# Bluear7878/Remote-Sensing-Vision-Language-Diffusion-Model

Measured on AMD Instinct MI355X. Metric: 512px x8 SR images/sec @50 steps, higher is better.
Workload: dtype f16 / bf16 MFMA operands as hi + lo pairs and triples, f32 accumulation and f32 residual streams (Stage 1: f16 tensors x f16 weight pairs; Stage 2: rsvld_amd.ops.UNET_POLICY; config.precision) -- the composition inside 1e-3 of the reference's CPU path (config.tolerance)

## Files before the change

include/rsvld_hip.h:

```cpp
#ifndef RSVLD_HIP_H
#define RSVLD_HIP_H

#include <stdint.h>

#ifdef __cplusplus
extern "C" {
#endif

#define RSVLD_OK 0
#define RSVLD_EINVAL (-1)
#define RSVLD_EUNSUPPORTED (-2)
#define RSVLD_ELAUNCH (-3)

#define RSVLD_F16 0
#define RSVLD_BF16 1
#define RSVLD_F32 2
#define RSVLD_SPLIT 3
#define RSVLD_F16W2 4
#define RSVLD_F16Q8 6
#define RSVLD_F16W1 5

#define RSVLD_ACT_NONE 0
#define RSVLD_ACT_SILU 1
#define RSVLD_ACT_GEGLU 2
// ... 167 lines not shown
int rsvld_llama_decode_attention(const void* qkv, const void* cos, const void* sin, const int64_t* pos, void* kcache, void* vcache, void* out,
                                 float* ws, int n_q, int n_kv, int head_dim, int max_len, float scale, int dtype, void* stream);

int rsvld_split_planes(const float* x, void* planes, int64_t rows, int C, void* stream);
int rsvld_merge_planes(const void* planes, float* x, int64_t rows, int C, void* stream);
int rsvld_planes_to_f16(const void* planes, int64_t ld, int64_t plane_stride, void* out_f16, int64_t out_ld, int64_t rows, int C, void* stream);
int rsvld_f16_to_planes(const void* x_f16, int64_t ld, void* planes, int64_t rows, int C, void* stream);
int rsvld_split_pack_weights(const float* w, void* w3, int64_t Cout, int taps, int Ctot, void* stream);
int rsvld_pack_weight_pairs(const float* w, void* w2, int64_t Cout, int taps, int Ctot, void* stream);
int rsvld_pack_weight_hq8(const float* w, void* whq, int64_t Cout, int taps, int Ctot, void* stream);
int rsvld_split_hq8(const float* x, void* out, int64_t rows, int C, void* stream);
int rsvld_planes_transpose_triple(const void* planes, void* w3, int64_t rows, int64_t rows_p, int C, int64_t ld, void* stream);
int rsvld_planes_to_triple(const void* planes, void* w3, int64_t rows, int64_t rows_p, int C, int64_t ld, void* stream);
int rsvld_softmax_rows_split(const float* s, void* p_planes, int64_t rows, int cols, int cols_p, int64_t ld, float scale, void* stream);
int rsvld_groupnorm_scale_shift_f32(const float* x, const float* x2, const float* gamma, const float* beta, float* scale_shift,
                                    int B, int HW, int C1, int C2, int groups, float eps, void* ws, void* stream);
int rsvld_groupnorm_stats_f32_fast(const float* x, const float* x2, float* mean_var, int B, int HW, int C1, int C2, int groups,
                                   void* ws, void* stream);
int rsvld_groupnorm_scale_shift_from_stats(const float* mean_var, const float* gamma, const float* beta, float* scale_shift,
                                           int B, int C, int groups, float eps, void* stream);
int rsvld_groupnorm_apply_split(const float* x, const float* x2, void* out, const float* scale_shift,
                                const float* mod_scale1p, const float* mod_shift, int mod_stride,
                                int B, int HW, int C1, int C2, int silu, int out_f32, void* stream);
int rsvld_layernorm_split(const float* x, void* out, const float* gamma, const float* beta, int64_t rows, int C, float eps,
                          int out_f32, void* stream);
int rsvld_attention_split_d64(const void* q, const void* k, const void* v, void* out, int B, int heads, int Nq, int Nk,
                              int64_t q_batch_stride, int64_t q_tok_stride, int64_t q_plane,
                              int64_t k_batch_stride, int64_t k_tok_stride, int64_t k_plane,
                              int64_t v_batch_stride, int64_t v_tok_stride, int64_t v_plane,
                              int64_t o_batch_stride, int64_t o_tok_stride, int64_t o_plane,
                              float scale, int out_f32, void* stream);
int rsvld_attention_split_d512_shared(const void* q, const void* x, void* out, int B, int Nq, int Nk,
                                      int64_t q_batch_stride, int64_t q_tok_stride, int64_t q_plane,
                                      int64_t x_batch_stride, int64_t x_tok_stride, int64_t x_plane,
                                      int64_t o_batch_stride, int64_t o_tok_stride, int64_t o_plane,
                                      float scale, int out_f32, void* stream);

#ifdef __cplusplus
}
#endif
#endif
```

remote-sensing-vision-language-diffusion-model_amd/_lib.py:

```python
import ctypes as C
import os

_PKG_DIR = os.path.dirname(os.path.abspath(__file__))
LIB_PATH = os.environ.get("RSVLD_LIB") or os.path.join(_PKG_DIR, "librsvld_hip.so")

F16, BF16, F32 = 0, 1, 2
SPLIT = 3
F16W2 = 4
F16W1 = 5
F16Q8 = 6
ACT_NONE, ACT_SILU, ACT_GEGLU = 0, 1, 2
TUNE_TILE = {"256x64": 1, "128x64": 2, "128x128": 3, "64x128": 4}
TUNE_STAGES_SHIFT, TUNE_NO_KSPLIT, TUNE_REG_STAGING = 3, 1 << 6, 1 << 7
TUNE_HALO_NW4, TUNE_HALO_NW8, TUNE_NO_GEMM256 = 1 << 8, 1 << 9, 1 << 10
TUNE_GEMM_ONE_TILE = 1 << 12
TUNE_F32_SPLIT = 1 << 11

ERRORS = {-1: "RSVLD_EINVAL (bad shape / pointer / combination)",
          -2: "RSVLD_EUNSUPPORTED", -3: "RSVLD_ELAUNCH (HIP launch failed)"}


class RsvldError(RuntimeError):
    pass

# ... 68 lines not shown
    "rsvld_concat_c_f32": (_i, [_vp, _vp, _vp, _i64, _i, _i, _vp]),
    "rsvld_axpby_f32": (_i, [_vp, _vp, _vp, _i64, _f, _f, _vp]),
    "rsvld_absdiff_sums_f32": (_i, [_vp, _vp, _vp, _i, _i64, _vp]),
    "rsvld_attention_f32": (_i, [_vp, _vp, _vp, _vp, _i, _i, _i, _i, _i,
                                 _i64, _i64, _i64, _i64, _i64, _i64, _i64, _i64, _f, _vp]),
    "rsvld_attention_f32_split": (_i, [_vp, _vp, _vp, _vp, _i, _i, _i, _i, _i,
                                 _i64, _i64, _i64, _i64, _i64, _i64, _i64, _i64, _f, _vp]),
    "rsvld_nchw_f32_to_nhwc_f32": (_i, [_vp, _vp, _i, _i, _i, _i, _i, _i, _i, _f, _vp]),
    "rsvld_split_planes": (_i, [_vp, _vp, _i64, _i, _vp]),
    "rsvld_merge_planes": (_i, [_vp, _vp, _i64, _i, _vp]),
    "rsvld_planes_to_f16": (_i, [_vp, _i64, _i64, _vp, _i64, _i64, _i, _vp]),
    "rsvld_f16_to_planes": (_i, [_vp, _i64, _vp, _i64, _i, _vp]),
    "rsvld_split_pack_weights": (_i, [_vp, _vp, _i64, _i, _i, _vp]),
    "rsvld_pack_weight_pairs": (_i, [_vp, _vp, _i64, _i, _i, _vp]),
    "rsvld_pack_weight_hq8": (_i, [_vp, _vp, _i64, _i, _i, _vp]),
    "rsvld_split_hq8": (_i, [_vp, _vp, _i64, _i, _vp]),
    "rsvld_planes_transpose_triple": (_i, [_vp, _vp, _i64, _i64, _i, _i64, _vp]),
    "rsvld_planes_to_triple": (_i, [_vp, _vp, _i64, _i64, _i, _i64, _vp]),
    "rsvld_softmax_rows_split": (_i, [_vp, _vp, _i64, _i, _i, _i64, _f, _vp]),
    "rsvld_groupnorm_scale_shift_f32": (_i, [_vp, _vp, _vp, _vp, _vp, _i, _i, _i, _i, _i, _f, _vp, _vp]),
    "rsvld_groupnorm_stats_f32_fast": (_i, [_vp, _vp, _vp, _i, _i, _i, _i, _i, _vp, _vp]),
    "rsvld_groupnorm_scale_shift_from_stats": (_i, [_vp, _vp, _vp, _vp, _i, _i, _i, _f, _vp]),
    "rsvld_groupnorm_apply_split": (_i, [_vp, _vp, _vp, _vp, _vp, _vp, _i, _i, _i, _i, _i, _i, _i, _vp]),
    "rsvld_layernorm_split": (_i, [_vp, _vp, _vp, _vp, _i64, _i, _f, _i, _vp]),
    "rsvld_attention_split_d512_shared": (_i, [_vp, _vp, _vp, _i, _i, _i, _i64, _i64, _i64, _i64, _i64, _i64, _i64, _i64, _i64, _f, _i, _vp]),
    "rsvld_attention_split_d64": (_i, [_vp, _vp, _vp, _vp, _i, _i, _i, _i,
                                       _i64, _i64, _i64, _i64, _i64, _i64, _i64, _i64, _i64, _i64, _i64, _i64, _f, _i, _vp]),
}

_lib = None


def load():
    global _lib
    if _lib is not None:
        return _lib
    import torch
    if not os.path.exists(LIB_PATH):
        raise RsvldError(
            f"{LIB_PATH} not found: build it with `python -c 'import __graft_entry__ as g; g.build()'` "
            f"(or `make -C {os.path.join(_PKG_DIR, 'csrc')}`). There is no CPU fallback.")
    lib = C.CDLL(LIB_PATH)
    for name, (res, args) in SIGNATURES.items():
        fn = getattr(lib, name)
        fn.restype = res
        fn.argtypes = args
# ... 8 lines not shown
```

remote-sensing-vision-language-diffusion-model_amd/csrc/norm.hip:

```cpp
#include "rsvld_common.h"

namespace {

template <typename T>
__global__ __launch_bounds__(256) void gn_partial_kernel(const T* __restrict__ x1, const T* __restrict__ x2,
                                                         float* __restrict__ part, int HW, int C1, int C2,
                                                         int groups, int rows_per_chunk, int nchunks) {
    extern __shared__ __attribute__((aligned(16))) char smem_raw[];
    float* sm = (float*)smem_raw;
    const int C = C1 + C2, C8 = C >> 3, C1_8 = C1 >> 3;
    const int TPR = C8 < 256 ? C8 : 256;
    const int rif = 256 / TPR;
    const int tid = threadIdx.x;
    const int chunk = blockIdx.x, b = blockIdx.y;
    const int row_lo = chunk * rows_per_chunk;
    const int row_hi = min(HW, row_lo + rows_per_chunk);
    const int tc = tid % TPR, rsub = tid / TPR;
    if (rsub < rif) {
        for (int cc = tc; cc < C8; cc += TPR) {
            float s[8], ss[8];
#pragma unroll
            for (int e = 0; e < 8; ++e) { s[e] = 0.f; ss[e] = 0.f; }
            const T* src;
            int64_t cstride;
// ... 57 lines not shown
        ss += __shfl_xor(ss, o);
    }
    if (lane == 0) {
        const double mean = s * inv_count;
        double var = ss * inv_count - mean * mean;
        if (var < 0.0) var = 0.0;
        stats[2 * i] = (float)mean;
        stats[2 * i + 1] = (float)var;
    }
}

template <bool PER_CHANNEL>
__global__ __launch_bounds__(256) void gn_ab_kernel(const float* __restrict__ part1, int n1, int C1,
                                                    const float* __restrict__ part2, int n2, int C2,
                                                    const float* __restrict__ gamma, const float* __restrict__ beta,
                                                    float* __restrict__ ab, float* __restrict__ stats_out, int groups,
                                                    float eps, double inv_count) {
    __shared__ double red[2][4];
    __shared__ float mr[2];
    const int g = blockIdx.x, b = blockIdx.y, tid = threadIdx.x;
    const int C = C1 + C2, gs = C / groups;
    double s = 0.0, ss = 0.0;
    if (PER_CHANNEL) {
        for (int c = g * gs; c < (g + 1) * gs; ++c) {
            const float* base;
            int n, Cs, cc;
            if (c < C1) { base = part1 + (int64_t)b * n1 * C1 * 2; n = n1; Cs = C1; cc = c; }
            else { base = part2 + (int64_t)b * n2 * C2 * 2; n = n2; Cs = C2; cc = c - C1; }
            for (int t = tid; t < n; t += 256) {
                s += (double)base[((int64_t)t * Cs + cc) * 2];
                ss += (double)base[((int64_t)t * Cs + cc) * 2 + 1];
            }
        }
    } else {
        for (int t = tid; t < n1; t += 256) {
            const float* q = part1 + (((int64_t)b * n1 + t) * groups + g) * 2;
            s += (double)q[0];
            ss += (double)q[1];
        }
    }
#pragma unroll
    for (int o = 32; o > 0; o >>= 1) { s += __shfl_xor(s, o); ss += __shfl_xor(ss, o); }
    if ((tid & 63) == 0) { red[0][tid >> 6] = s; red[1][tid >> 6] = ss; }
    __syncthreads();
    if (tid == 0) {
        s = red[0][0] + red[0][1] + red[0][2] + red[0][3];
        ss = red[1][0] + red[1][1] + red[1][2] + red[1][3];
        const double mean = s * inv_count;
        double var = ss * inv_count - mean * mean;
        if (var < 0.0) var = 0.0;
        mr[0] = (float)mean;
        mr[1] = (float)var;
        if (stats_out != nullptr) {
            stats_out[((int64_t)b * groups + g) * 2] = (float)mean;
// ... 218 lines not shown
#pragma unroll
            for (int e = 0; e < 8; ++e) {
                const float t = f[e] * sa[e] + sb[e];
                f[e] = silu ? silu_f(t) : t;
            }
            *(u32x4*)(dst + (int64_t)(row0 + i * rstep) * C) = pack8<T>(f);
        }
}


__device__ __forceinline__ void ld8f(const float* p, float (&f)[8]) {
    const f32x4 a = *(const f32x4*)p, b = *(const f32x4*)(p + 4);
    f[0] = a[0]; f[1] = a[1]; f[2] = a[2]; f[3] = a[3]; f[4] = b[0]; f[5] = b[1]; f[6] = b[2]; f[7] = b[3];
}
__device__ __forceinline__ void st_planes8(bf16* row, int C, int c, const float (&f)[8]) {
    bf16x8 hv;
    float lo[8];
#pragma unroll
    for (int e = 0; e < 8; ++e) { hv[e] = (bf16)f[e]; lo[e] = f[e] - (float)hv[e]; }
    *(u32x4*)(row + c) = pack8<bf16>(lo);
    *(u32x4*)(row + C + c) = __builtin_bit_cast(u32x4, hv);
}

__global__ __launch_bounds__(256) void gn_partial_f32_kernel(const float* __restrict__ x1, const float* __restrict__ x2,
                                                             float* __restrict__ part, int HW, int C1, int C2, int groups,
                                                             int rows_per_chunk, int nchunks) {
    extern __shared__ __attribute__((aligned(16))) char smem_raw[];
    float* sm = (float*)smem_raw;
    const int C = C1 + C2, C8 = C >> 3, C1_8 = C1 >> 3;
    const int TPR = C8 < 256 ? C8 : 256, rif = 256 / TPR;
    const int tid = threadIdx.x, chunk = blockIdx.x, b = blockIdx.y;
    const int row_lo = chunk * rows_per_chunk, row_hi = min(HW, row_lo + rows_per_chunk);
    const int tc = tid % TPR, rsub = tid / TPR;
    if (rsub < rif) {
        for (int cc = tc; cc < C8; cc += TPR) {
            float s[8], ss[8];
#pragma unroll
            for (int e = 0; e < 8; ++e) { s[e] = 0.f; ss[e] = 0.f; }
            const float* src;
            int64_t cstride;
            int coff;
            if (cc < C1_8) { src = x1 + (int64_t)b * HW * C1; cstride = C1; coff = cc * 8; }
            else { src = x2 + (int64_t)b * HW * C2; cstride = C2; coff = (cc - C1_8) * 8; }
            int r = row_lo + rsub;
            for (; r + rif < row_hi; r += 2 * rif) {
                float f0[8], f1[8];
                ld8f(src + (int64_t)r * cstride + coff, f0);
                ld8f(src + (int64_t)(r + rif) * cstride + coff, f1);
#pragma unroll
                for (int e = 0; e < 8; ++e) { s[e] += f0[e]; ss[e] += f0[e] * f0[e]; }
#pragma unroll
                for (int e = 0; e < 8; ++e) { s[e] += f1[e]; ss[e] += f1[e] * f1[e]; }
            }
            for (; r < row_hi; r += rif) {
                float f[8];
                ld8f(src + (int64_t)r * cstride + coff, f);
#pragma unroll
                for (int e = 0; e < 8; ++e) { s[e] += f[e]; ss[e] += f[e] * f[e]; }
            }
            float* dst = sm + ((int64_t)rsub * C + cc * 8) * 2;
#pragma unroll
            for (int e = 0; e < 8; ++e) { dst[2 * e] = s[e]; dst[2 * e + 1] = ss[e]; }
        }
    }
    __syncthreads();
    const int gs = C / groups;
    for (int g = tid; g < groups; g += 256) {
        float s = 0.f, ss = 0.f;
        for (int r = 0; r < rif; ++r) {
            const float* src = sm + ((int64_t)r * C + g * gs) * 2;
            for (int e = 0; e < gs; ++e) { s += src[2 * e]; ss += src[2 * e + 1]; }
        }
        float* o = part + (((int64_t)b * nchunks + chunk) * groups + g) * 2;
        o[0] = s;
        o[1] = ss;
    }
}

template <int OUT>
__global__ __launch_bounds__(256) void gn_apply_split_kernel(const float* __restrict__ x1, const float* __restrict__ x2, void* __restrict__ y,
                                                             const float* __restrict__ ab, const float* __restrict__ mod_scale,
                                                             const float* __restrict__ mod_shift, int HW, int C1, int C2, int silu,
                                                             int rows_per_block, int mod_stride) {
    const int C = C1 + C2, C8 = C >> 3, C1_8 = C1 >> 3;
    const int TPR = C8 < 256 ? C8 : 256, rif = 256 / TPR;
    const int tid = threadIdx.x, tc = tid % TPR, rsub = tid / TPR;
    if (rsub >= rif) return;
    const int b = blockIdx.y;
    const int row_lo = blockIdx.x * rows_per_block, row_hi = min(HW, row_lo + rows_per_block);
    for (int cc = tc; cc < C8; cc += TPR) {
        float sa[8], sb[8];
        {
            const float* a = ab + ((int64_t)b * C + cc * 8) * 2;
#pragma unroll
            for (int e = 0; e < 8; ++e) { sa[e] = a[2 * e]; sb[e] = a[2 * e + 1]; }
        }
        const float* src;
        int64_t cstride;
        int coff;
        if (cc < C1_8) { src = x1 + (int64_t)b * HW * C1; cstride = C1; coff = cc * 8; }
        else { src = x2 + (int64_t)b * HW * C2; cstride = C2; coff = (cc - C1_8) * 8; }
        auto emit = [&](int r, float (&f)[8]) {
#pragma unroll
            for (int e = 0; e < 8; ++e) {
                const float t = f[e] * sa[e] + sb[e];
                f[e] = silu ? silu_f(t) : t;
            }
            if (mod_scale != nullptr) {
                const int64_t mo = ((int64_t)b * HW + r) * mod_stride + cc * 8;
                float ms[8], mh[8];
                ld8f(mod_scale + mo, ms);
                ld8f(mod_shift + mo, mh);
#pragma unroll
                for (int e = 0; e < 8; ++e) f[e] = f[e] * (1.f + ms[e]) + mh[e];
            }
            const int64_t pix = (int64_t)b * HW + r;
            if (OUT == 1) {
                float* o = (float*)y + pix * C + cc * 8;
                *(f32x4*)o = (f32x4){f[0], f[1], f[2], f[3]};
                *(f32x4*)(o + 4) = (f32x4){f[4], f[5], f[6], f[7]};
            } else if (OUT == 2) {
                *(u32x4*)((f16*)y + pix * C + cc * 8) = pack8<f16>(f);
            } else if (OUT == 3) {
                st_hq8<true, RSVLD_HQ8_SX_LO, RSVLD_HQ8_SX_HI>((f16*)y + pix * (2 * (int64_t)C), C, cc * 8, f);
            } else {
                st_planes8((bf16*)y + pix * (2 * C), C, cc * 8, f);
            }
        };
        int r = row_lo + rsub;
        for (; r + rif < row_hi; r += 2 * rif) {
            float f0[8], f1[8];
            ld8f(src + (int64_t)r * cstride + coff, f0);
            ld8f(src + (int64_t)(r + rif) * cstride + coff, f1);
            emit(r, f0);
            emit(r + rif, f1);
        }
        for (; r < row_hi; r += rif) {
            float f[8];
            ld8f(src + (int64_t)r * cstride + coff, f);
            emit(r, f);
        }
    }
}

template <int MAXC, int ROWS, int OUT>
__global__ __launch_bounds__(256) void layernorm_split_kernel(const float* __restrict__ x, void* __restrict__ y,
                                                              const float* __restrict__ gamma, const float* __restrict__ beta,
                                                              int64_t rows, int C, float eps) {
    const int lane = threadIdx.x & 63;
    const int C8 = C >> 3;
    float ga[MAXC][8], be[MAXC][8];
#pragma unroll
    for (int j = 0; j < MAXC; ++j) {
        const int cc = lane + 64 * j;
#pragma unroll
        for (int e = 0; e < 8; ++e) {
            ga[j][e] = (gamma != nullptr && cc < C8) ? gamma[cc * 8 + e] : 1.f;
            be[j][e] = (beta != nullptr && cc < C8) ? beta[cc * 8 + e] : 0.f;
        }
    }
    const int64_t wave_id = (int64_t)blockIdx.x * 4 + (threadIdx.x >> 6);
    const int64_t nwaves = (int64_t)gridDim.x * 4;
    for (int64_t row0 = wave_id * ROWS; row0 < rows; row0 += nwaves * ROWS) {
        float f[ROWS][MAXC][8];
// ... 58 lines not shown
    const float a = (gamma ? gamma[c] : 1.f) * (1.0f / sqrtf(var + eps));
    ab[2 * (int64_t)i] = a;
    ab[2 * (int64_t)i + 1] = (beta ? beta[c] : 0.f) - mean * a;
}

bool gn_small_ok(int B, int HW, int C1, int C2, int groups) {
    const int C = C1 + C2, gs = C / groups;
    if (gs % 8) return false;
    const int gs8 = gs / 8;
    if (gs8 > 256 || (gs8 & (gs8 - 1))) return false;
    if (C2 > 0 && C1 % gs) return false;
    if ((int64_t)HW * gs8 > (int64_t)256 * GN_SMALL_MAXV) return false;
    (void)B;
    return groups >= 32;
}

struct GnPlan {
    int nchunks, rows_per_chunk;
};
GnPlan gn_plan(int B, int HW) {
    (void)B;
    const int max_chunks = 512;
    int rpc = (HW + max_chunks - 1) / max_chunks;
    if (rpc < 64) rpc = 64;
    GnPlan p;
    p.rows_per_chunk = rpc;
    p.nchunks = (HW + rpc - 1) / rpc;
    return p;
}

bool gn_shape_ok(int B, int HW, int C1, int C2, int groups) {
    if (B <= 0 || HW <= 0 || C1 <= 0 || C1 % 8 || C2 < 0 || C2 % 8 || groups <= 0) return false;
    const int C = C1 + C2;
    if (C % groups) return false;
    if (C > 8192 || groups > 256) return false;
    return true;
}

template <typename T>
int gn_stats_impl(const void* x, const void* x2, float* stats, int B, int HW, int C1, int C2, int groups, void* ws,
                  hipStream_t s) {
    const GnPlan pl = gn_plan(B, HW);
    const int C = C1 + C2, C8 = C / 8;
    const int TPR = C8 < 256 ? C8 : 256, rif = 256 / TPR;
    const size_t smem = (size_t)rif * C * 2 * sizeof(float);
    float* part = (float*)ws;
// ... 140 lines not shown
    }
}

extern "C" int rsvld_layernorm(const void* x, void* y, const float* gamma, const float* beta, int64_t rows, int C,
                               float eps, int dtype, void* stream) {
    if (!x || !y || rows <= 0 || C <= 0 || C % 8 || C > 4096) return RSVLD_EINVAL;
    hipStream_t s = (hipStream_t)stream;
    if (dtype == RSVLD_F16) launch_layernorm<f16>(x, y, gamma, beta, rows, C, eps, s);
    else if (dtype == RSVLD_BF16) launch_layernorm<bf16>(x, y, gamma, beta, rows, C, eps, s);
    else return RSVLD_EINVAL;
    return rsvld_check_launch();
}

extern "C" int rsvld_groupnorm_scale_shift_f32(const float* x, const float* x2, const float* gamma, const float* beta,
                                               float* scale_shift, int B, int HW, int C1, int C2, int groups, float eps, void* ws,
                                               void* stream) {
    if (!x || !ws || !scale_shift || !gn_shape_ok(B, HW, C1, C2, groups) || ((C2 > 0) != (x2 != nullptr)) || B > 65535) return RSVLD_EINVAL;
    hipStream_t s = (hipStream_t)stream;
    const GnPlan pl = gn_plan(B, HW);
    const int C = C1 + C2, C8 = C / 8;
    const int TPR = C8 < 256 ? C8 : 256, rif = 256 / TPR;
    const size_t smem = (size_t)rif * C * 2 * sizeof(float);
    float* part = (float*)ws;
    hipLaunchKernelGGL(gn_partial_f32_kernel, dim3(pl.nchunks, B), dim3(256), smem, s, x, x2, part, HW, C1, C2, groups,
                       pl.rows_per_chunk, pl.nchunks);
    const double inv_count = 1.0 / ((double)HW * (double)(C / groups));
    hipLaunchKernelGGL(gn_ab_kernel<false>, dim3(groups, B), dim3(256), 0, s, part, pl.nchunks, C, nullptr, 0, 0, gamma, beta,
                       scale_shift, nullptr, groups, eps, inv_count);
    return rsvld_check_launch();
}

extern "C" int rsvld_groupnorm_apply_split(const float* x, const float* x2, void* out, const float* scale_shift,
                                           const float* mod_scale1p, const float* mod_shift, int mod_stride, int B, int HW, int C1,
                                           int C2, int silu, int out_f32, void* stream) {
    if (!x || !out || !scale_shift || B <= 0 || B > 65535 || HW <= 0 || C1 <= 0 || C1 % 8 || C2 < 0 || C2 % 8 || ((C2 > 0) != (x2 != nullptr)))
        return RSVLD_EINVAL;
    if ((mod_scale1p != nullptr) != (mod_shift != nullptr) || mod_stride < 0 || (mod_stride & 3)) return RSVLD_EINVAL;
    const int C = C1 + C2, C8 = C / 8;
    const int TPR = C8 < 256 ? C8 : 256, rif = 256 / TPR;
    int max_blocks = 2048 / B;
    if (max_blocks < 1) max_blocks = 1;
    int rpb = (HW + max_blocks - 1) / max_blocks;
    if (rpb < 2 * rif) rpb = 2 * rif;
    const int nblk = (HW + rpb - 1) / rpb;
    hipStream_t s = (hipStream_t)stream;
    if (out_f32 < 0 || out_f32 > 3 || (out_f32 == 3 && (C1 + C2) % 32)) return RSVLD_EINVAL;
    if (out_f32 == 3)
        hipLaunchKernelGGL(gn_apply_split_kernel<3>, dim3((unsigned)nblk, B), dim3(256), 0, s, x, x2, out, scale_shift, mod_scale1p,
                           mod_shift, HW, C1, C2, silu, rpb, mod_stride > 0 ? mod_stride : C);
    else if (out_f32 == 1)
        hipLaunchKernelGGL(gn_apply_split_kernel<1>, dim3((unsigned)nblk, B), dim3(256), 0, s, x, x2, out, scale_shift, mod_scale1p,
                           mod_shift, HW, C1, C2, silu, rpb, mod_stride > 0 ? mod_stride : C);
    else if (out_f32 == 2)
        hipLaunchKernelGGL(gn_apply_split_kernel<2>, dim3((unsigned)nblk, B), dim3(256), 0, s, x, x2, out, scale_shift, mod_scale1p,
                           mod_shift, HW, C1, C2, silu, rpb, mod_stride > 0 ? mod_stride : C);
    else
        hipLaunchKernelGGL(gn_apply_split_kernel<0>, dim3((unsigned)nblk, B), dim3(256), 0, s, x, x2, out, scale_shift, mod_scale1p,
                           mod_shift, HW, C1, C2, silu, rpb, mod_stride > 0 ? mod_stride : C);
    return rsvld_check_launch();
}

template <int OUT_F32>
static void launch_layernorm_split(const float* x, void* y, const float* gamma, const float* beta, int64_t rows, int C, float eps,
                                   hipStream_t s) {
    const int chunks_per_lane = (C / 8 + 63) / 64;
    auto blocks = [&](int rows_per_block) {
        const int64_t n = cdiv64(rows, rows_per_block);
        return (unsigned)(n < 768 ? n : 768);
    };
    if (chunks_per_lane <= 2) hipLaunchKernelGGL((layernorm_split_kernel<2, 2, OUT_F32>), dim3(blocks(8)), dim3(256), 0, s, x, y, gamma, beta, rows, C, eps);
    else if (chunks_per_lane == 3) hipLaunchKernelGGL((layernorm_split_kernel<3, 2, OUT_F32>), dim3(blocks(8)), dim3(256), 0, s, x, y, gamma, beta, rows, C, eps);
    else if (chunks_per_lane <= 4) hipLaunchKernelGGL((layernorm_split_kernel<4, 1, OUT_F32>), dim3(blocks(4)), dim3(256), 0, s, x, y, gamma, beta, rows, C, eps);
    else hipLaunchKernelGGL((layernorm_split_kernel<8, 1, OUT_F32>), dim3(blocks(4)), dim3(256), 0, s, x, y, gamma, beta, rows, C, eps);
}

extern "C" int rsvld_layernorm_split(const float* x, void* out, const float* gamma, const float* beta, int64_t rows, int C, float eps,
                                     int out_f32, void* stream) {
    if (!x || !out || rows <= 0 || C <= 0 || C % 8 || C > 4096) return RSVLD_EINVAL;
    hipStream_t s = (hipStream_t)stream;
    if (out_f32 < 0 || out_f32 > 2) return RSVLD_EINVAL;
    if (out_f32 == 1) launch_layernorm_split<1>(x, out, gamma, beta, rows, C, eps, s);
    else if (out_f32 == 2) launch_layernorm_split<2>(x, out, gamma, beta, rows, C, eps, s);
    else launch_layernorm_split<0>(x, out, gamma, beta, rows, C, eps, s);
    return rsvld_check_launch();
}

extern "C" int rsvld_groupnorm_stats_f32_fast(const float* x, const float* x2, float* mean_var, int B, int HW, int C1, int C2, int groups,
                                              void* ws, void* stream) {
    if (!x || !mean_var || !ws || !gn_shape_ok(B, HW, C1, C2, groups) || ((C2 > 0) != (x2 != nullptr)) || B > 65535) return RSVLD_EINVAL;
    hipStream_t s = (hipStream_t)stream;
    const GnPlan pl = gn_plan(B, HW);
    const int C = C1 + C2, C8 = C / 8;
    const int TPR = C8 < 256 ? C8 : 256, rif = 256 / TPR;
    const size_t smem = (size_t)rif * C * 2 * sizeof(float);
    float* part = (float*)ws;
    hipLaunchKernelGGL(gn_partial_f32_kernel, dim3(pl.nchunks, B), dim3(256), smem, s, x, x2, part, HW, C1, C2, groups,
                       pl.rows_per_chunk, pl.nchunks);
    const int total = B * groups;
    const double inv_count = 1.0 / ((double)HW * (double)(C / groups));
    hipLaunchKernelGGL(gn_finalize_kernel, dim3((total + 3) / 4), dim3(256), 0, s, part, mean_var, groups, pl.nchunks, inv_count, total);
    return rsvld_check_launch();
}

extern "C" int rsvld_groupnorm_scale_shift_from_stats(const float* mean_var, const float* gamma, const float* beta, float* scale_shift,
                                                      int B, int C, int groups, float eps, void* stream) {
    if (!mean_var || !scale_shift || B <= 0 || C <= 0 || groups <= 0 || C % groups) return RSVLD_EINVAL;
    const int total = B * C;
    hipLaunchKernelGGL(gn_ab_from_stats_kernel, dim3((total + 255) / 256), dim3(256), 0, (hipStream_t)stream, mean_var, gamma, beta,
                       scale_shift, C, groups, eps, total);
    return rsvld_check_launch();
}
```

remote-sensing-vision-language-diffusion-model_amd/ops.py:

```python
import contextlib
import ctypes as C
import contextvars
import math

import torch

from . import _lib as L

_DT = {torch.float16: L.F16, torch.bfloat16: L.BF16}


def _stream():
    return C.c_void_p(torch.cuda.current_stream().cuda_stream)


def _ptr(t):
    return None if t is None else C.c_void_p(t.data_ptr())


def _need_gpu(*ts):
    for t in ts:
        if t is not None and not t.is_cuda:
            raise L.RsvldError("rsvld_amd ops run on the GPU only (got a CPU tensor); there is no CPU fallback")

# ... 685 lines not shown
    lib = L.load()
    if not lib.rsvld_conv3x3_halo_supported(C.byref(d)):
        raise L.RsvldError("conv2d (q8): shape not supported by the halo kernel (checked by _q8_conv_eligible)")
    part_out, ntiles = None, ((H + 7) // 8) * ((W + 31) // 32)
    if stats:
        part_out = torch.empty((B, ntiles, pc.cout_p, 2), device=out.device, dtype=torch.float32)
    flops = 2.0 * B * H * W * pc.cout * pc.cin * 9
    nbytes = 4.0 * (B * H * W * Cc + out.numel() + (0 if residual is None else residual.numel())) + 4.0 * pc.w.numel()
    _launch("conv_halo_128_q8" + _detail(B, H, W, Cc, 0, pc, 1, False), flops, nbytes, lambda: L.check(
        lib.rsvld_conv3x3_halo_nhwc(C.byref(d), None, 0, _ptr(part_out), _stream()), "rsvld_conv3x3_halo_nhwc"))
    if part_out is not None:
        out._gn_part = (part_out, ntiles)
    out._nhwc = True
    return out


def _gn_scale_shift_f32(x, x2, gamma, nbeta, groups, eps):
    B, H, W, C1 = x.shape
    C2 = 0 if x2 is None else x2.shape[-1]
    lib = L.load()
    ab = torch.empty((B, C1 + C2, 2), device=x.device, dtype=torch.float32)
    part1 = getattr(x, "_gn_part", None)
    part2 = None if x2 is None else getattr(x2, "_gn_part", None)
    if part1 is not None and (x2 is None or part2 is not None):
        _launch("groupnorm_ab_from_partials", 0.0, 0.0, lambda: L.check(lib.rsvld_groupnorm_scale_shift_from_partials(
            _ptr(part1[0]), part1[1], C1, None if part2 is None else _ptr(part2[0]), 0 if part2 is None else part2[1],
            C2, _ptr(gamma), _ptr(nbeta), _ptr(ab), B, H * W, groups, eps, _stream()), "rsvld_groupnorm_scale_shift_from_partials"))
        return ab
    if not x.is_contiguous() or (x2 is not None and not x2.is_contiguous()):
        raise L.RsvldError("group_norm (split): contiguous fp32 NHWC inputs expected")
    ws = torch.empty(lib.rsvld_groupnorm_ws_bytes(B, H * W, C1 + C2, groups), device=x.device, dtype=torch.uint8)
    _launch("groupnorm_stats_split", 0.0, 4.0 * (x.numel() + (0 if x2 is None else x2.numel())), lambda: L.check(
        lib.rsvld_groupnorm_scale_shift_f32(_ptr(x), _ptr(x2), _ptr(gamma), _ptr(nbeta), _ptr(ab), B, H * W, C1, C2, groups, eps,
                                            _ptr(ws), _stream()), "rsvld_groupnorm_scale_shift_f32"))
    return ab


def _gn_apply_split(x, x2, ab, silu, planes, mod_scale1p=None, mod_shift=None, f16=False, q8=False):
    B, H, W, C1 = x.shape
    C2 = 0 if x2 is None else x2.shape[-1]
    Cc = C1 + C2
    mod_stride = 0
    if mod_scale1p is not None:
        mod_stride = mod_scale1p.stride(-2)
        if (mod_shift.stride(-2) != mod_stride or mod_scale1p.stride(-1) != 1 or mod_shift.stride(-1) != 1
                or mod_scale1p.dtype != torch.float32 or mod_shift.dtype != torch.float32):
            raise L.RsvldError("group_norm: modulation tensors must be fp32, share a row stride and be channel-contiguous")
    f16 = f16 and planes
    if q8:
        out = torch.empty((B, H, W, 2, Cc), device=x.device, dtype=torch.float16)
        _launch("groupnorm_apply_q8", 0.0, 8.0 * B * H * W * Cc, lambda: L.check(L.load().rsvld_groupnorm_apply_split(
            _ptr(x), _ptr(x2), _ptr(out), _ptr(ab), _ptr(mod_scale1p), _ptr(mod_shift), mod_stride, B, H * W, C1, C2, int(silu), 3, _stream()),
            "rsvld_groupnorm_apply_split"))
        return Q8Rows(out)
    if f16:
        out = torch.empty((B, H, W, Cc), device=x.device, dtype=torch.float16)
    elif planes:
        out = torch.empty((B, H, W, 2, Cc), device=x.device, dtype=torch.bfloat16)
    else:
        out = torch.empty((B, H, W, Cc), device=x.device, dtype=torch.float32)
    _launch("groupnorm_apply_split", 0.0, (6.0 if f16 else 8.0) * B * H * W * Cc, lambda: L.check(L.load().rsvld_groupnorm_apply_split(
        _ptr(x), _ptr(x2), _ptr(out), _ptr(ab), _ptr(mod_scale1p), _ptr(mod_shift), mod_stride, B, H * W, C1, C2, int(silu),
        2 if f16 else int(not planes), _stream()), "rsvld_groupnorm_apply_split"))
    if f16:
        return out
    if planes:
        return Planes(out)
    out._nhwc = True
    return out


def _detail(B, Ho, Wo, Cin, Cin2, pc, stride, upsample):
    if not _CTX.get().profile_detail:
        return ""
    return f" [{B}x{Ho}x{Wo} {Cin}+{Cin2}->{pc.cout_p} k{pc.kh} s{stride}{' up' if upsample else ''}]"


def _conv2d_split(x, pc, *, x2, stride, pad, upsample, rowvec, residual, act, alpha, beta, norm, stats, out_planes, out_group=None,
                  norm_group=None, group=None):

    if norm is not None:
        gamma, nbeta, groups, eps, silu = norm
        if isinstance(x, Planes) or isinstance(x2, Planes):
            raise L.RsvldError("conv2d (split): norm= needs the fp32 tensors")
        ab = _gn_scale_shift_f32(x, x2, gamma, nbeta, groups, eps)
        if f16_group(norm_group):
            x16 = _gn_apply_split(x, x2, ab, silu, planes=True, f16=True)
            return conv2d(x16, pc, stride=stride, pad=pad, upsample=upsample, rowvec=rowvec, residual=residual, act=act, alpha=alpha,
                          beta=beta, stats=stats, out_planes=out_planes, out_group=out_group, group=group)
        if q8_group(norm_group) and _q8_conv_eligible(x.shape[0], x.shape[1], x.shape[2], x.shape[3] + (0 if x2 is None else x2.shape[3]), pc,
                                                      stride, pad, upsample, act, out_planes):
            return _conv2d_q8(_gn_apply_split(x, x2, ab, silu, planes=True, q8=True), pc, rowvec=rowvec, residual=residual, alpha=alpha,
# ... 722 lines not shown
```

remote-sensing-vision-language-diffusion-model_amd/sgm/modules/diffusionmodules/openaimodel.py:

```python
import torch
from torch import nn

from .... import ops
from ....hipnn import HipNet
from ...util import default, exists
from ..attention import SpatialTransformer
from .util import conv_nd, linear, normalization, timestep_embedding, zero_module


class TimestepBlock(nn.Module):
    """Marker: ``run(rt, x, emb_rows)`` takes the timestep embedding."""


class TimestepEmbedSequential(nn.Sequential, TimestepBlock):
    def run(self, rt, x, emb_rows, context=None):
        for layer in self:
            if isinstance(layer, TimestepBlock):
                x = layer.run(rt, x, emb_rows)
            elif isinstance(layer, SpatialTransformer):
                x = layer.run(rt, x, context)
            elif isinstance(layer, nn.Conv2d):
                x = ops.conv2d(x, rt.pk(layer), pad=layer.padding[0])
            else:
                x = layer.run(rt, x)
# ... 39 lines not shown
        self.out_layers = nn.Sequential(normalization(self.out_channels), nn.SiLU(), nn.Dropout(p=dropout),
                                        zero_module(conv_nd(dims, self.out_channels, self.out_channels, kernel_size,
                                                            padding=pad)))
        if self.out_channels == channels:
            self.skip_connection = nn.Identity()
        elif use_conv:
            self.skip_connection = conv_nd(dims, channels, self.out_channels, kernel_size, padding=pad)
        else:
            self.skip_connection = conv_nd(dims, channels, self.out_channels, 1)

    @property
    def _emb_linear(self):
        return self.emb_layers[1]

    def run(self, rt, x, emb_rows):
        gn1, conv1 = self.in_layers[0], self.in_layers[2]
        gn2, conv2 = self.out_layers[0], self.out_layers[3]
        h = ops.conv2d(x, rt.pk(conv1), pad=conv1.padding[0], rowvec=emb_rows[id(self)], stats=True,
                       norm=(gn1.weight, gn1.bias, gn1.num_groups, gn1.eps, True), norm_group="conv1")
        if isinstance(self.skip_connection, nn.Conv2d):
            skip = ops.conv2d(x, rt.pk(self.skip_connection), pad=self.skip_connection.padding[0])
        else:
            skip = x
        return ops.conv2d(h, rt.pk(conv2), pad=conv2.padding[0], residual=skip,
                          norm=(gn2.weight, gn2.bias, gn2.num_groups, gn2.eps, True), norm_group="conv2")


class UNetModel(HipNet):

    def __init__(self, in_channels, model_channels, out_channels, num_res_blocks, attention_resolutions, dropout=0,
                 channel_mult=(1, 2, 4, 8), conv_resample=True, dims=2, num_classes=None, use_checkpoint=False,
                 use_fp16=False, num_heads=-1, num_head_channels=-1, num_heads_upsample=-1,
                 use_scale_shift_norm=False, resblock_updown=False, use_new_attention_order=False,
                 use_spatial_transformer=False, transformer_depth=1, context_dim=None, n_embed=None, legacy=True,
                 disable_self_attentions=None, num_attention_blocks=None, disable_middle_self_attn=False,
                 use_linear_in_transformer=False, spatial_transformer_attn_type="softmax", adm_in_channels=None,
                 use_fairscale_checkpoint=False, offload_to_cpu=False, transformer_depth_middle=None, **ignored):
        super().__init__()
        if not use_spatial_transformer or context_dim is None:
            raise NotImplementedError("the SR networks are SDXL UNets with spatial transformers")
        if resblock_updown or use_scale_shift_norm or n_embed is not None or dims != 2:
            raise NotImplementedError("option not used by juggernautXL.yaml")
        if num_heads == -1 and num_head_channels == -1:
            raise ValueError("Either num_heads or num_head_channels has to be set")
        channel_mult = list(channel_mult)
        if isinstance(context_dim, (list, tuple)):
            context_dim = list(context_dim)
# ... 100 lines not shown
```

Before: 0.01361.

## Fuse per-channel GroupNorm statistics into apply and conv epilogues, retune LayerNorm

The fp32 GroupNorm apply kernel now writes per-block per-channel sum and sum-of-squares partials, and the second ResBlock conv also requests stats. A following GroupNorm can then build scale and shift from these partials and skip a full re-read of the activation. When only one of two concatenated sources carries partials, the other source gets a partials-only pass. The partials reducer is vectorised and unrolled, and small-C LayerNorm gets a new wave-per-row-group kernel. The cost is extra partial-buffer writes and shared-memory reductions in the apply kernel, plus several interacting code paths to keep correct.

```diff
diff --git a/include/rsvld_hip.h b/include/rsvld_hip.h
--- a/include/rsvld_hip.h
+++ b/include/rsvld_hip.h
@@ -213,6 +213,11 @@
 int rsvld_groupnorm_apply_split(const float* x, const float* x2, void* out, const float* scale_shift,
                                 const float* mod_scale1p, const float* mod_shift, int mod_stride,
                                 int B, int HW, int C1, int C2, int silu, int out_f32, void* stream);
+int rsvld_groupnorm_row_blocks(int HW);
+int rsvld_groupnorm_apply_split_stats(const float* x, const float* x2, float* out, const float* scale_shift,
+                                      const float* mod_scale1p, const float* mod_shift, int mod_stride,
+                                      int B, int HW, int C1, int C2, int silu, float* part_out, void* stream);
+int rsvld_groupnorm_partials_f32(const float* x, float* part, int B, int HW, int C, void* stream);
 int rsvld_layernorm_split(const float* x, void* out, const float* gamma, const float* beta, int64_t rows, int C, float eps,
                           int out_f32, void* stream);
 int rsvld_attention_split_d64(const void* q, const void* k, const void* v, void* out, int B, int heads, int Nq, int Nk,
diff --git a/remote-sensing-vision-language-diffusion-model_amd/_lib.py b/remote-sensing-vision-language-diffusion-model_amd/_lib.py
--- a/remote-sensing-vision-language-diffusion-model_amd/_lib.py
+++ b/remote-sensing-vision-language-diffusion-model_amd/_lib.py
@@ -114,6 +114,9 @@
     "rsvld_groupnorm_stats_f32_fast": (_i, [_vp, _vp, _vp, _i, _i, _i, _i, _i, _vp, _vp]),
     "rsvld_groupnorm_scale_shift_from_stats": (_i, [_vp, _vp, _vp, _vp, _i, _i, _i, _f, _vp]),
     "rsvld_groupnorm_apply_split": (_i, [_vp, _vp, _vp, _vp, _vp, _vp, _i, _i, _i, _i, _i, _i, _i, _vp]),
+    "rsvld_groupnorm_row_blocks": (_i, [_i]),
+    "rsvld_groupnorm_apply_split_stats": (_i, [_vp, _vp, _vp, _vp, _vp, _vp, _i, _i, _i, _i, _i, _i, _vp, _vp]),
+    "rsvld_groupnorm_partials_f32": (_i, [_vp, _vp, _i, _i, _i, _vp]),
     "rsvld_layernorm_split": (_i, [_vp, _vp, _vp, _vp, _i64, _i, _f, _i, _vp]),
     "rsvld_attention_split_d512_shared": (_i, [_vp, _vp, _vp, _i, _i, _i, _i64, _i64, _i64, _i64, _i64, _i64, _i64, _i64, _i64, _f, _i, _vp]),
     "rsvld_attention_split_d64": (_i, [_vp, _vp, _vp, _vp, _i, _i, _i, _i,
diff --git a/remote-sensing-vision-language-diffusion-model_amd/csrc/norm.hip b/remote-sensing-vision-language-diffusion-model_amd/csrc/norm.hip
--- a/remote-sensing-vision-language-diffusion-model_amd/csrc/norm.hip
+++ b/remote-sensing-vision-language-diffusion-model_amd/csrc/norm.hip
@@ -103,14 +103,28 @@
     const int C = C1 + C2, gs = C / groups;
     double s = 0.0, ss = 0.0;
     if (PER_CHANNEL) {
-        for (int c = g * gs; c < (g + 1) * gs; ++c) {
-            const float* base;
-            int n, Cs, cc;
-            if (c < C1) { base = part1 + (int64_t)b * n1 * C1 * 2; n = n1; Cs = C1; cc = c; }
-            else { base = part2 + (int64_t)b * n2 * C2 * 2; n = n2; Cs = C2; cc = c - C1; }
-            for (int t = tid; t < n; t += 256) {
-                s += (double)base[((int64_t)t * Cs + cc) * 2];
-                ss += (double)base[((int64_t)t * Cs + cc) * 2 + 1];
+        const int W = gs < 256 ? gs : 256, nsub = 256 / W;
+        const int cl = tid % W, rsub = tid / W;
+        if (rsub < nsub) {
+            for (int c = g * gs + cl; c < (g + 1) * gs; c += W) {
+                const f32x2_t* p;
+                int n;
+                int64_t Cs;
+                if (c < C1) { p = (const f32x2_t*)part1 + (int64_t)b * n1 * C1 + c; n = n1; Cs = C1; }
+                else { p = (const f32x2_t*)part2 + (int64_t)b * n2 * C2 + (c - C1); n = n2; Cs = C2; }
+                int t = rsub;
+                for (; t + 3 * nsub < n; t += 4 * nsub) {
+                    f32x2_t v[4];
+#pragma unroll
+                    for (int u = 0; u < 4; ++u) v[u] = p[(int64_t)(t + u * nsub) * Cs];
+#pragma unroll
+                    for (int u = 0; u < 4; ++u) { s += (double)v[u][0]; ss += (double)v[u][1]; }
+                }
+                for (; t < n; t += nsub) {
+                    const f32x2_t v = p[(int64_t)t * Cs];
+                    s += (double)v[0];
+                    ss += (double)v[1];
+                }
             }
         }
     } else {
@@ -375,6 +389,7 @@
     *(u32x4*)(row + C + c) = __builtin_bit_cast(u32x4, hv);
 }
 
+template <bool PER_CHANNEL>
 __global__ __launch_bounds__(256) void gn_partial_f32_kernel(const float* __restrict__ x1, const float* __restrict__ x2,
                                                              float* __restrict__ part, int HW, int C1, int C2, int groups,
                                                              int rows_per_chunk, int nchunks) {
@@ -417,6 +432,15 @@
         }
     }
     __syncthreads();
+    if (PER_CHANNEL) {
+        float* o = part + ((int64_t)b * nchunks + chunk) * C * 2;
+        for (int i = tid; i < 2 * C; i += 256) {
+            float a = 0.f;
+            for (int r = 0; r < rif; ++r) a += sm[(int64_t)r * C * 2 + i];
+            o[i] = a;
+        }
+        return;
+    }
     const int gs = C / groups;
     for (int g = tid; g < groups; g += 256) {
         float s = 0.f, ss = 0.f;
@@ -430,18 +454,23 @@
     }
 }
 
-template <int OUT>
+template <int OUT, bool STATS>
 __global__ __launch_bounds__(256) void gn_apply_split_kernel(const float* __restrict__ x1, const float* __restrict__ x2, void* __restrict__ y,
                                                              const float* __restrict__ ab, const float* __restrict__ mod_scale,
-                                                             const float* __restrict__ mod_shift, int HW, int C1, int C2, int silu,
-                                                             int rows_per_block, int mod_stride) {
+                                                             const float* __restrict__ mod_shift, float* __restrict__ part_out, int HW,
+                                                             int C1, int C2, int silu, int rows_per_block, int mod_stride) {
+    static_assert(!STATS || OUT == 1, "statistics are those of the fp32 output");
+    __shared__ __attribute__((aligned(16))) float sm_part[STATS ? 256 * 16 : 1];
     const int C = C1 + C2, C8 = C >> 3, C1_8 = C1 >> 3;
     const int TPR = C8 < 256 ? C8 : 256, rif = 256 / TPR;
     const int tid = threadIdx.x, tc = tid % TPR, rsub = tid / TPR;
-    if (rsub >= rif) return;
+    if (!STATS && rsub >= rif) return;
     const int b = blockIdx.y;
     const int row_lo = blockIdx.x * rows_per_block, row_hi = min(HW, row_lo + rows_per_block);
-    for (int cc = tc; cc < C8; cc += TPR) {
+    for (int cc = tc; rsub < rif && cc < C8; cc += TPR) {
+        float ps[8], pss[8];
+#pragma unroll
+        for (int e = 0; e < 8; ++e) { ps[e] = 0.f; pss[e] = 0.f; }
         float sa[8], sb[8];
         {
             const float* a = ab + ((int64_t)b * C + cc * 8) * 2;
@@ -466,6 +495,10 @@
                 ld8f(mod_shift + mo, mh);
 #pragma unroll
                 for (int e = 0; e < 8; ++e) f[e] = f[e] * (1.f + ms[e]) + mh[e];
+            }
+            if (STATS) {
+#pragma unroll
+                for (int e = 0; e < 8; ++e) { ps[e] += f[e]; pss[e] += f[e] * f[e]; }
             }
             const int64_t pix = (int64_t)b * HW + r;
             if (OUT == 1) {
@@ -493,6 +526,26 @@
             ld8f(src + (int64_t)r * cstride + coff, f);
             emit(r, f);
         }
+        if (STATS) {
+            if (rif == 1) {
+                float* o = part_out + (((int64_t)b * gridDim.x + blockIdx.x) * C + cc * 8) * 2;
+#pragma unroll
+                for (int e = 0; e < 8; e += 2) *(f32x4*)(o + 2 * e) = (f32x4){ps[e], pss[e], ps[e + 1], pss[e + 1]};
+            } else {
+                float* o = sm_part + (rsub * C + cc * 8) * 2;
+#pragma unroll
+                for (int e = 0; e < 8; e += 2) *(f32x4*)(o + 2 * e) = (f32x4){ps[e], pss[e], ps[e + 1], pss[e + 1]};
+            }
+        }
+    }
+    if (STATS && rif > 1) {
+        __syncthreads();
+        float* o = part_out + ((int64_t)b * gridDim.x + blockIdx.x) * C * 2;
+        for (int i = tid; i < 2 * C; i += 256) {
+            float a = 0.f;
+            for (int r = 0; r < rif; ++r) a += sm_part[r * C * 2 + i];
+            o[i] = a;
+        }
     }
 }
 
@@ -597,6 +650,15 @@
     (void)B;
     const int max_chunks = 512;
     int rpc = (HW + max_chunks - 1) / max_chunks;
+    if (rpc < 64) rpc = 64;
+    GnPlan p;
+    p.rows_per_chunk = rpc;
+    p.nchunks = (HW + rpc - 1) / rpc;
+    return p;
+}
+
+GnPlan gn_pc_plan(int HW) {
+    int rpc = (HW + 2047) / 2048;
     if (rpc < 64) rpc = 64;
     GnPlan p;
     p.rows_per_chunk = rpc;
@@ -783,7 +845,7 @@
     const int TPR = C8 < 256 ? C8 : 256, rif = 256 / TPR;
     const size_t smem = (size_t)rif * C * 2 * sizeof(float);
     float* part = (float*)ws;
-    hipLaunchKernelGGL(gn_partial_f32_kernel, dim3(pl.nchunks, B), dim3(256), smem, s, x, x2, part, HW, C1, C2, groups,
+    hipLaunchKernelGGL(gn_partial_f32_kernel<false>, dim3(pl.nchunks, B), dim3(256), smem, s, x, x2, part, HW, C1, C2, groups,
                        pl.rows_per_chunk, pl.nchunks);
     const double inv_count = 1.0 / ((double)HW * (double)(C / groups));
     hipLaunchKernelGGL(gn_ab_kernel<false>, dim3(groups, B), dim3(256), 0, s, part, pl.nchunks, C, nullptr, 0, 0, gamma, beta,
@@ -807,18 +869,123 @@
     hipStream_t s = (hipStream_t)stream;
     if (out_f32 < 0 || out_f32 > 3 || (out_f32 == 3 && (C1 + C2) % 32)) return RSVLD_EINVAL;
     if (out_f32 == 3)
-        hipLaunchKernelGGL(gn_apply_split_kernel<3>, dim3((unsigned)nblk, B), dim3(256), 0, s, x, x2, out, scale_shift, mod_scale1p,
-                           mod_shift, HW, C1, C2, silu, rpb, mod_stride > 0 ? mod_stride : C);
+        hipLaunchKernelGGL((gn_apply_split_kernel<3, false>), dim3((unsigned)nblk, B), dim3(256), 0, s, x, x2, out, scale_shift, mod_scale1p,
+                           mod_shift, nullptr, HW, C1, C2, silu, rpb, mod_stride > 0 ? mod_stride : C);
     else if (out_f32 == 1)
-        hipLaunchKernelGGL(gn_apply_split_kernel<1>, dim3((unsigned)nblk, B), dim3(256), 0, s, x, x2, out, scale_shift, mod_scale1p,
-                           mod_shift, HW, C1, C2, silu, rpb, mod_stride > 0 ? mod_stride : C);
+        hipLaunchKernelGGL((gn_apply_split_kernel<1, false>), dim3((unsigned)nblk, B), dim3(256), 0, s, x, x2, out, scale_shift, mod_scale1p,
+                           mod_shift, nullptr, HW, C1, C2, silu, rpb, mod_stride > 0 ? mod_stride : C);
     else if (out_f32 == 2)
-        hipLaunchKernelGGL(gn_apply_split_kernel<2>, dim3((unsigned)nblk, B), dim3(256), 0, s, x, x2, out, scale_shift, mod_scale1p,
-                           mod_shift, HW, C1, C2, silu, rpb, mod_stride > 0 ? mod_stride : C);
+        hipLaunchKernelGGL((gn_apply_split_kernel<2, false>), dim3((unsigned)nblk, B), dim3(256), 0, s, x, x2, out, scale_shift, mod_scale1p,
+                           mod_shift, nullptr, HW, C1, C2, silu, rpb, mod_stride > 0 ? mod_stride : C);
     else
-        hipLaunchKernelGGL(gn_apply_split_kernel<0>, dim3((unsigned)nblk, B), dim3(256), 0, s, x, x2, out, scale_shift, mod_scale1p,
-                           mod_shift, HW, C1, C2, silu, rpb, mod_stride > 0 ? mod_stride : C);
-    return rsvld_check_launch();
+        hipLaunchKernelGGL((gn_apply_split_kernel<0, false>), dim3((unsigned)nblk, B), dim3(256), 0, s, x, x2, out, scale_shift, mod_scale1p,
+                           mod_shift, nullptr, HW, C1, C2, silu, rpb, mod_stride > 0 ? mod_stride : C);
+    return rsvld_check_launch();
+}
+
+extern "C" int rsvld_groupnorm_row_blocks(int HW) { return HW > 0 ? gn_pc_plan(HW).nchunks : 0; }
+
+extern "C" int rsvld_groupnorm_apply_split_stats(const float* x, const float* x2, float* out, const float* scale_shift,
+                                                 const float* mod_scale1p, const float* mod_shift, int mod_stride, int B, int HW, int C1,
+                                                 int C2, int silu, float* part_out, void* stream) {
+    if (!x || !out || !scale_shift || !part_out || B <= 0 || B > 65535 || HW <= 0 || C1 <= 0 || C1 % 8 || C2 < 0 || C2 % 8 ||
+        ((C2 > 0) != (x2 != nullptr)))
+        return RSVLD_EINVAL;
+    if ((mod_scale1p != nullptr) != (mod_shift != nullptr) || mod_stride < 0 || (mod_stride & 3)) return RSVLD_EINVAL;
+    const GnPlan pl = gn_pc_plan(HW);
+    hipLaunchKernelGGL((gn_apply_split_kernel<1, true>), dim3((unsigned)pl.nchunks, B), dim3(256), 0, (hipStream_t)stream, x, x2, (void*)out,
+                       scale_shift, mod_scale1p, mod_shift, part_out, HW, C1, C2, silu, pl.rows_per_chunk, mod_stride > 0 ? mod_stride : C1 + C2);
+    return rsvld_check_launch();
+}
+
+extern "C" int rsvld_groupnorm_partials_f32(const float* x, float* part, int B, int HW, int C, void* stream) {
+    if (!x || !part || B <= 0 || B > 65535 || HW <= 0 || C <= 0 || C % 8 || C > 8192) return RSVLD_EINVAL;
+    const GnPlan pl = gn_pc_plan(HW);
+    const int C8 = C / 8, TPR = C8 < 256 ? C8 : 256, rif = 256 / TPR;
+    const size_t smem = (size_t)rif * C * 2 * sizeof(float);
+    hipLaunchKernelGGL(gn_partial_f32_kernel<true>, dim3(pl.nchunks, B), dim3(256), smem, (hipStream_t)stream, x, (const float*)nullptr, part, HW,
+                       C, 0, 1, pl.rows_per_chunk, pl.nchunks);
+    return rsvld_check_launch();
+}
+
+namespace {
+template <int LPR, int NP, int ROWS, int OUT>
+__global__ __launch_bounds__(256) void layernorm_split_p4_kernel(const float* __restrict__ x, void* __restrict__ y,
+                                                                 const float* __restrict__ gamma, const float* __restrict__ beta,
+                                                                 int64_t rows, int C, float eps) {
+    constexpr int SUBS = 64 / LPR;
+    const int lane = threadIdx.x & 63, l = lane & (LPR - 1), sub = lane / LPR;
+    const int C4 = C >> 2;
+    f32x4 ga[NP], be[NP];
+#pragma unroll
+    for (int j = 0; j < NP; ++j) {
+        const int p = l + LPR * j;
+#pragma unroll
+        for (int e = 0; e < 4; ++e) {
+            ga[j][e] = (gamma != nullptr && p < C4) ? gamma[p * 4 + e] : 1.f;
+            be[j][e] = (beta != nullptr && p < C4) ? beta[p * 4 + e] : 0.f;
+        }
+    }
+    const int64_t wave_id = (int64_t)blockIdx.x * 4 + (threadIdx.x >> 6);
+    const int64_t nwaves = (int64_t)gridDim.x * 4;
+    for (int64_t row0 = wave_id * (SUBS * ROWS); row0 < rows; row0 += nwaves * (SUBS * ROWS)) {
+        f32x4 f[ROWS][NP];
+#pragma unroll
+        for (int r = 0; r < ROWS; ++r)
+#pragma unroll
+            for (int j = 0; j < NP; ++j) {
+                const int p = l + LPR * j;
+                const int64_t row = row0 + r * SUBS + sub;
+                f[r][j] = (p < C4 && row < rows) ? *(const f32x4*)(x + row * C + p * 4) : (f32x4){0.f, 0.f, 0.f, 0.f};
+            }
+#pragma unroll
+        for (int r = 0; r < ROWS; ++r) {
+            const int64_t row = row0 + r * SUBS + sub;
+            float s = 0.f;
+#pragma unroll
+            for (int j = 0; j < NP; ++j)
+                if (l + LPR * j < C4) s += (f[r][j][0] + f[r][j][1]) + (f[r][j][2] + f[r][j][3]);
+#pragma unroll
+            for (int o = LPR / 2; o > 0; o >>= 1) s += __shfl_xor(s, o);
+            const float mean = s / (float)C;
+            float ss = 0.f;
+#pragma unroll
+            for (int j = 0; j < NP; ++j)
+                if (l + LPR * j < C4) {
+#pragma unroll
+                    for (int e = 0; e < 4; ++e) { const float d = f[r][j][e] - mean; ss += d * d; }
+                }
+#pragma unroll
+            for (int o = LPR / 2; o > 0; o >>= 1) ss += __shfl_xor(ss, o);
+            const float rstd = 1.0f / sqrtf(ss / (float)C + eps);
+            if (row < rows) {
+#pragma unroll
+                for (int j = 0; j < NP; ++j) {
+                    const int p = l + LPR * j;
+                    if (p < C4) {
+                        f32x4 o;
+#pragma unroll
+                        for (int e = 0; e < 4; ++e) o[e] = (f[r][j][e] - mean) * rstd * ga[j][e] + be[j][e];
+                        if (OUT == 1) {
+                            *(f32x4*)((float*)y + row * C + p * 4) = o;
+                        } else if (OUT == 2) {
+                            const f16x4 h = {(f16)o[0], (f16)o[1], (f16)o[2], (f16)o[3]};
+                            *(u32x2*)((f16*)y + row * C + p * 4) = __builtin_bit_cast(u32x2, h);
+                        } else {
+                            bf16x4 hv, lv;
+#pragma unroll
+                            for (int e = 0; e < 4; ++e) { hv[e] = (bf16)o[e]; lv[e] = (bf16)(o[e] - (float)hv[e]); }
+                            bf16* d = (bf16*)y + row * (2 * (int64_t)C) + p * 4;
+                            *(u32x2*)d = __builtin_bit_cast(u32x2, lv);
+                            *(u32x2*)(d + C) = __builtin_bit_cast(u32x2, hv);
+                        }
+                    }
+                }
+            }
+        }
+    }
+}
+
 }
 
 template <int OUT_F32>
@@ -827,9 +994,10 @@
     const int chunks_per_lane = (C / 8 + 63) / 64;
     auto blocks = [&](int rows_per_block) {
         const int64_t n = cdiv64(rows, rows_per_block);
-        return (unsigned)(n < 768 ? n : 768);
+        return (unsigned)(n <= 768 ? n : cdiv64(n, cdiv64(n, 768)));
     };
-    if (chunks_per_lane <= 2) hipLaunchKernelGGL((layernorm_split_kernel<2, 2, OUT_F32>), dim3(blocks(8)), dim3(256), 0, s, x, y, gamma, beta, rows, C, eps);
+    if (C <= 640) hipLaunchKernelGGL((layernorm_split_p4_kernel<32, 5, 2, OUT_F32>), dim3(blocks(16)), dim3(256), 0, s, x, y, gamma, beta, rows, C, eps);
+    else if (C <= 1280) hipLaunchKernelGGL((layernorm_split_p4_kernel<64, 5, 2, OUT_F32>), dim3(blocks(8)), dim3(256), 0, s, x, y, gamma, beta, rows, C, eps);
     else if (chunks_per_lane == 3) hipLaunchKernelGGL((layernorm_split_kernel<3, 2, OUT_F32>), dim3(blocks(8)), dim3(256), 0, s, x, y, gamma, beta, rows, C, eps);
     else if (chunks_per_lane <= 4) hipLaunchKernelGGL((layernorm_split_kernel<4, 1, OUT_F32>), dim3(blocks(4)), dim3(256), 0, s, x, y, gamma, beta, rows, C, eps);
     else hipLaunchKernelGGL((layernorm_split_kernel<8, 1, OUT_F32>), dim3(blocks(4)), dim3(256), 0, s, x, y, gamma, beta, rows, C, eps);
@@ -855,7 +1023,7 @@
     const int TPR = C8 < 256 ? C8 : 256, rif = 256 / TPR;
     const size_t smem = (size_t)rif * C * 2 * sizeof(float);
     float* part = (float*)ws;
-    hipLaunchKernelGGL(gn_partial_f32_kernel, dim3(pl.nchunks, B), dim3(256), smem, s, x, x2, part, HW, C1, C2, groups,
+    hipLaunchKernelGGL(gn_partial_f32_kernel<false>, dim3(pl.nchunks, B), dim3(256), smem, s, x, x2, part, HW, C1, C2, groups,
                        pl.rows_per_chunk, pl.nchunks);
     const int total = B * groups;
     const double inv_count = 1.0 / ((double)HW * (double)(C / groups));
diff --git a/remote-sensing-vision-language-diffusion-model_amd/ops.py b/remote-sensing-vision-language-diffusion-model_amd/ops.py
--- a/remote-sensing-vision-language-diffusion-model_amd/ops.py
+++ b/remote-sensing-vision-language-diffusion-model_amd/ops.py
@@ -731,18 +731,40 @@
     ab = torch.empty((B, C1 + C2, 2), device=x.device, dtype=torch.float32)
     part1 = getattr(x, "_gn_part", None)
     part2 = None if x2 is None else getattr(x2, "_gn_part", None)
+    if not x.is_contiguous() or (x2 is not None and not x2.is_contiguous()):
+        raise L.RsvldError("group_norm (split): contiguous fp32 NHWC inputs expected")
+    if x2 is not None and (part1 is None) != (part2 is None):
+        if part1 is None:
+            part1 = _gn_partials_f32(x)
+        else:
+            part2 = _gn_partials_f32(x2)
     if part1 is not None and (x2 is None or part2 is not None):
         _launch("groupnorm_ab_from_partials", 0.0, 0.0, lambda: L.check(lib.rsvld_groupnorm_scale_shift_from_partials(
             _ptr(part1[0]), part1[1], C1, None if part2 is None else _ptr(part2[0]), 0 if part2 is None else part2[1],
             C2, _ptr(gamma), _ptr(nbeta), _ptr(ab), B, H * W, groups, eps, _stream()), "rsvld_groupnorm_scale_shift_from_partials"))
         return ab
-    if not x.is_contiguous() or (x2 is not None and not x2.is_contiguous()):
-        raise L.RsvldError("group_norm (split): contiguous fp32 NHWC inputs expected")
     ws = torch.empty(lib.rsvld_groupnorm_ws_bytes(B, H * W, C1 + C2, groups), device=x.device, dtype=torch.uint8)
-    _launch("groupnorm_stats_split", 0.0, 4.0 * (x.numel() + (0 if x2 is None else x2.numel())), lambda: L.check(
+    _launch("groupnorm_stats_split" + _gn_detail(x, x2), 0.0, 4.0 * (x.numel() + (0 if x2 is None else x2.numel())), lambda: L.check(
         lib.rsvld_groupnorm_scale_shift_f32(_ptr(x), _ptr(x2), _ptr(gamma), _ptr(nbeta), _ptr(ab), B, H * W, C1, C2, groups, eps,
                                             _ptr(ws), _stream()), "rsvld_groupnorm_scale_shift_f32"))
     return ab
+
+
+def _gn_detail(x, x2, note=""):
+    if not _CTX.get().profile_detail:
+        return ""
+    B, H, W, C1 = x.shape
+    return f" [{B}x{H}x{W} {C1}+{0 if x2 is None else x2.shape[-1]}{note}]"
+
+
+def _gn_partials_f32(x):
+    B, H, W, Cc = x.shape
+    lib = L.load()
+    nblk = lib.rsvld_groupnorm_row_blocks(H * W)
+    part = torch.empty((B, nblk, Cc, 2), device=x.device, dtype=torch.float32)
+    _launch("groupnorm_stats_split" + _gn_detail(x, None, " one of two sources"), 0.0, 4.0 * x.numel(), lambda: L.check(
+        lib.rsvld_groupnorm_partials_f32(_ptr(x), _ptr(part), B, H * W, Cc, _stream()), "rsvld_groupnorm_partials_f32"))
+    return part, nblk
 
 
 def _gn_apply_split(x, x2, ab, silu, planes, mod_scale1p=None, mod_shift=None, f16=False, q8=False):
@@ -767,16 +789,20 @@
     elif planes:
         out = torch.empty((B, H, W, 2, Cc), device=x.device, dtype=torch.bfloat16)
     else:
+        lib = L.load()
         out = torch.empty((B, H, W, Cc), device=x.device, dtype=torch.float32)
+        nblk = lib.rsvld_groupnorm_row_blocks(H * W)
+        part_out = torch.empty((B, nblk, Cc, 2), device=x.device, dtype=torch.float32)
+        _launch("groupnorm_apply_split", 0.0, 8.0 * B * H * W * Cc, lambda: L.check(lib.rsvld_groupnorm_apply_split_stats(
+            _ptr(x), _ptr(x2), _ptr(out), _ptr(ab), _ptr(mod_scale1p), _ptr(mod_shift), mod_stride, B, H * W, C1, C2, int(silu),
+            _ptr(part_out), _stream()), "rsvld_groupnorm_apply_split_stats"))
+        out._gn_part = (part_out, nblk)
+        out._nhwc = True
+        return out
     _launch("groupnorm_apply_split", 0.0, (6.0 if f16 else 8.0) * B * H * W * Cc, lambda: L.check(L.load().rsvld_groupnorm_apply_split(
         _ptr(x), _ptr(x2), _ptr(out), _ptr(ab), _ptr(mod_scale1p), _ptr(mod_shift), mod_stride, B, H * W, C1, C2, int(silu),
-        2 if f16 else int(not planes), _stream()), "rsvld_groupnorm_apply_split"))
-    if f16:
-        return out
-    if planes:
-        return Planes(out)
-    out._nhwc = True
-    return out
+        2 if f16 else 0, _stream()), "rsvld_groupnorm_apply_split"))
+    return out if f16 else Planes(out)
 
 
 def _detail(B, Ho, Wo, Cin, Cin2, pc, stride, upsample):
diff --git a/remote-sensing-vision-language-diffusion-model_amd/sgm/modules/diffusionmodules/openaimodel.py b/remote-sensing-vision-language-diffusion-model_amd/sgm/modules/diffusionmodules/openaimodel.py
--- a/remote-sensing-vision-language-diffusion-model_amd/sgm/modules/diffusionmodules/openaimodel.py
+++ b/remote-sensing-vision-language-diffusion-model_amd/sgm/modules/diffusionmodules/openaimodel.py
@@ -85,7 +85,7 @@
             skip = ops.conv2d(x, rt.pk(self.skip_connection), pad=self.skip_connection.padding[0])
         else:
             skip = x
-        return ops.conv2d(h, rt.pk(conv2), pad=conv2.padding[0], residual=skip,
+        return ops.conv2d(h, rt.pk(conv2), pad=conv2.padding[0], residual=skip, stats=True,
                           norm=(gn2.weight, gn2.bias, gn2.num_groups, gn2.eps, True), norm_group="conv2")
 
 
```

Result: no change. 0.01359 (-0.2%).
